# KorAP/Datok

Measured on AMD Instinct MI355X. Metric: input MB/s tokenized, tokenizer_de.matok, higher is better.
Workload: dtype u32 table cells, u8 symbol codes; 1 GPU; tokenizer_de.matok, 4096 equal-length 4096 B synthetic German docs per batch (BASELINE.json configs[1]); table_layout=matrix: state-major fused u32 cells, docs_per_gpu=4096, doc_bytes=4096, parallelism=documents sharded over 1 GPU(s), no data-path collective, batches_in_flight=3, inputs=one per batch in flight (generator seeds 2, 3, 4 on rank 0)

## Files before the change

### datok_amd/_lib.py

```python
import ctypes as C
import os
import subprocess

_HERE = os.path.dirname(os.path.abspath(__file__))
LIB_PATH = os.environ.get("DATOK_GPU_LIB") or os.path.join(_HERE, "libdatok_gpu.so")

OK, E_IO, E_FORMAT, E_NO_DEVICE, E_HIP, E_ARG, E_MODEL, E_CAPACITY, E_STATE, E_NOMEM = 0, -1, -2, -3, -4, -5, -6, -7, -8, -9
ST_WINDOW_OVERFLOW, ST_EMPTY_TEXT, ST_BAD_MODEL, ST_IRREGULAR, ST_STEP_LIMIT, ST_INTERNAL = 1, 2, 4, 8, 16, 32
ST_BAD_OFFSET = 64

EXPORTS = [
    "dtk_device_count", "dtk_set_device", "dtk_strerror", "dtk_last_hip_error",
    "dtk_model_load", "dtk_model_load_mem", "dtk_model_free", "dtk_model_type", "dtk_model_get_info",
    "dtk_model_info_mem",
    "dtk_batch_create", "dtk_batch_free", "dtk_batch_set_input", "dtk_batch_set_input_device",
    "dtk_batch_run", "dtk_batch_sync", "dtk_batch_stream", "dtk_batch_totals",
    "dtk_batch_set_profiling", "dtk_batch_stage_ms", "dtk_batch_set_chunking", "dtk_batch_set_warm_extend",
    "dtk_batch_result_device", "dtk_batch_result_host", "dtk_transduce", "dtk_free",
    "dtk_foma_to_matok", "dtk_foma_to_datok", "dtk_transduce_replay", "dtk_batch_render_device", "dtk_batch_render_host",
    "dtk_batch_status_host", "dtk_transduce_release", "dtk_transduce_result",
    "dtk_pipeline_create", "dtk_pipeline_free", "dtk_pipeline_set_chunking", "dtk_pipeline_run",
    "dtk_pinned_alloc", "dtk_pinned_free",
    "dtk_batch_set_result_fields", "dtk_batch_download_begin", "dtk_pipeline_set_result_fields",
    "dtk_batch_set_download_stream", "dtk_batch_download_stream", "dtk_batch_done", "dtk_batch_set_streams",
    "dtk_debug_configure", "dtk_batch_debug_stream", "dtk_blk_start", "dtk_blk_end",
    "dtk_multi_create", "dtk_multi_free", "dtk_multi_type", "dtk_multi_set_result_fields", "dtk_multi_set_chunking", "dtk_multi_run",
]


class ModelInfo(C.Structure):
    _fields_ = [("kind", C.c_int32), ("epsilon", C.c_int32), ("unknown", C.c_int32),
                ("identity", C.c_int32), ("final_state", C.c_int32), ("sigma_count", C.c_int32),
                ("state_count", C.c_uint32), ("array_len", C.c_uint64),
                ("n_eps_states", C.c_uint32), ("max_eps_chain", C.c_uint32),
                ("entry_bytes", C.c_uint32), ("device_bytes", C.c_uint64),
                ("unknown_used", C.c_uint32), ("dense_states", C.c_uint32),
                ("stream_codes", C.c_uint32)]


class Totals(C.Structure):
# ... 117 lines not shown
    L.dtk_multi_free.argtypes = [vp]
    L.dtk_multi_free.restype = None
    L.dtk_multi_type.argtypes = [vp]
    L.dtk_multi_type.restype = C.c_char_p
    L.dtk_multi_set_result_fields.argtypes = [vp, u32]
    L.dtk_multi_set_chunking.argtypes = [vp, u32, u32]
    L.dtk_multi_run.argtypes = [vp, vp, vp, u32, u32, SLICE_FN, vp]
    for f in (L.dtk_blk_start, L.dtk_blk_end):
        f.argtypes, f.restype = [vp, vp, u64], C.c_int32
    L.dtk_pinned_alloc.restype = vp
    L.dtk_pinned_alloc.argtypes = [sz]
    L.dtk_pinned_free.argtypes = [vp]
    L.dtk_pinned_free.restype = None
    L.dtk_debug_configure.argtypes = [C.c_char_p, C.c_char_p]
    L.dtk_batch_debug_stream.argtypes = [vp, vp, vp, C.POINTER(u32)]
    for k, v in os.environ.items():
        if k.startswith("DATOK_") and k not in ("DATOK_GPU_LIB", "DATOK_GATHER_TIMEOUT"):
            L.dtk_debug_configure(k.encode(), v.encode())
    _lib = L
    return L


def check(code, what=""):
    if code != OK:
        raise DatokGpuError(code, what)
```

### datok_amd/csrc/dtk_batch.cpp

```cpp
#include <algorithm>
#include <cstdio>
#include <cstring>
#include <memory>

#include "dtk_host.h"

static int alloc_outputs(dtk_batch *b, uint64_t tok, uint64_t sent, uint64_t text) {
  auto grow = [](auto &a, uint64_t n) { return a.fit(n, std::max<uint64_t>(n, 4)); };
  int rc;
  if (tok > b->tok_cap) {
    b->tok_cap = 0;
    if ((rc = grow(b->d_rstart, tok)) || (rc = grow(b->d_rend, tok)) || (rc = grow(b->d_bstart, tok)) ||
        (rc = grow(b->d_bend, tok)) || (rc = grow(b->d_sbefore, tok)))
      return rc;
    b->tok_cap = tok;
  }
  if (sent > b->sent_cap) {
    b->sent_cap = 0;
    if ((rc = grow(b->d_sent, sent))) return rc;
    b->sent_cap = sent;
  }
  if (text > b->text_cap) {
    b->text_cap = 0;
    if ((rc = grow(b->d_ttok, text)) || (rc = grow(b->d_tsent, text)) || (rc = grow(b->d_ts_end, text))) return rc;
// ... 6 lines not shown
  if (!out || max_docs == 0) return DTK_E_ARG;
  *out = nullptr;
  if (dtk_device_count() <= 0) return DTK_E_NO_DEVICE;
  std::unique_ptr<dtk_batch> b(new dtk_batch());
  b->max_bytes = max_bytes;
  b->max_docs = max_docs;
  HIP_TRY(hipGetDevice(&b->device));
  int rc = b->stream.create();
  if (rc != DTK_OK) return rc;
  if (g_dbg.round_limit >= 0) b->round_limit = (uint32_t)g_dbg.round_limit;
  const uint64_t pad = 256, nd1 = (uint64_t)max_docs + 1;
  auto make = [](auto &a, uint64_t n) { return a.fit(n, n); };
  if ((rc = make(b->d_text_own, max_bytes + pad)) || (rc = make(b->d_off_own, nd1)) ||
      (rc = make(b->d_sym, max_bytes + pad)) || (rc = make(b->d_rsbits, (max_bytes + pad) / 8 + 64)) ||
      (rc = make(b->d_bits, EVB_KINDS * ((max_bytes + max_docs) / 32 + 8) + 8)) ||
      (rc = make(b->d_acc, DTK_TOTALS_BYTES + 3 * nd1 * 8 + 4 * (uint64_t)max_docs * 4 + 64)) ||
      (rc = make(b->d_redo, max_docs)) || (rc = make(b->d_blk_doc, max_bytes / DTK_SYM_BLOCK_BYTES + 3)) ||
      (rc = make(b->d_chunk_off, nd1)) || (rc = make(b->d_big_docs, nd1)) ||
      (rc = make(b->d_csr, 3 * nd1)) || (rc = make(b->d_doc_ns, nd1)) ||
      (rc = make(b->d_scan_ws, ((uint64_t)max_docs / 2048 + 2) * 4)) || (rc = make(b->d_out_off, nd1)) ||
      (rc = b->h_totals_pin.fit(DTK_TOTALS_BYTES, DTK_TOTALS_BYTES)) || (rc = b->h_off_pin.fit(nd1 * 8, nd1 * 8)))
    return rc;
  b->d_tok_off = b->d_csr; b->d_sent_off = b->d_csr + nd1; b->d_text_off = b->d_csr + 2 * nd1;
  b->h_totals = b->h_totals_pin.as<DtkTotalsDev>();
  rc = alloc_outputs(b.get(), max_bytes / 3 + max_docs + 16, max_bytes / 8 + 2ull * max_docs + 16,
                     max_bytes / 64 + 2ull * max_docs + 16);
  if (rc != DTK_OK) return rc;
  *out = b.release();
  return DTK_OK;
}

// ... 307 lines not shown
  }
  b->last_model = m;
  b->last_flags = flags;
  b->repair_rounds = 0;
  hipStream_t s = b->stream;
  const bool prof = b->profiling;
#define STAGE(i) do { if (prof) HIP_TRY(hipEventRecord(b->ev[i], s)); } while (0)
  STAGE(0);
  bool fold_acc = false;
  size_t acc_bytes = 0;
  {
    const size_t nd = b->n_docs;
    uint8_t *q = b->d_acc;
    b->d_tok_off = b->d_csr; b->d_sent_off = b->d_csr + (nd + 1); b->d_text_off = b->d_csr + 2 * (nd + 1);
    b->d_totals = (DtkTotalsDev *)q; q += DTK_TOTALS_BYTES;
    b->d_tok_cnt = (uint64_t *)q; q += (nd + 1) * 8;
    b->d_sent_cnt = (uint64_t *)q; q += (nd + 1) * 8;
    b->d_text_cnt = (uint64_t *)q; q += (nd + 1) * 8;
    b->d_status = (uint32_t *)q; q += nd * 4;
    b->d_first_bad = (uint32_t *)q; q += nd * 4;
    b->d_fail_lane = (uint32_t *)q; q += nd * 4;
    b->d_doc_tail = (uint32_t *)q; q += nd * 4;
    const size_t acc_used = ((size_t)(q - b->d_acc) + 15) & ~(size_t)15;
    b->bit_words = (uint32_t)(((b->total + nd) / 32 + 8) & ~(uint64_t)3);
    const bool fold = b->total > 0;
    fold_acc = fold && b->acc_primed && acc_used / 16 < 0xFFFFFFFFull && !g_dbg.clear_kernel;
    if (!fold_acc) {
      if (dtk_launch_clear2(b->d_acc, acc_used, b->d_bits, fold ? 0 : (size_t)EVB_KINDS * b->bit_words * 4, s))
        return hip_fail(hipGetLastError(), "clear");
      b->acc_primed = true;
    }
    acc_bytes = acc_used;
  }
  STAGE(1);
  if (dtk_launch_symbolize(b->d_text, b->d_off, b->n_docs, b->total, &m->sig, b->d_sym,
                           b->d_text == b->d_text_own, b->d_blk_doc, (unsigned long long *)&b->d_totals->invalid_epoch,
                           (uint32_t *)b->d_rsbits.p, b->d_bits, b->bit_words, fold_acc ? b->d_acc.p : nullptr, acc_bytes,
                           ++b->epoch, s))
    return hip_fail(hipGetLastError(), "symbolize");
  STAGE(2);
  DtkWalkArgs w = walk_args(b);
  bool fix_in_scan = false;
  DtkSpecArgs sp_first{};
  if (b->chunk == 0) {
    STAGE(3); STAGE(4);
    if (dtk_launch_walk(&m->tab, &w, s)) return hip_fail(hipGetLastError(), "walk");
    STAGE(5); STAGE(6); STAGE(7);
  } else {
    DtkSpecArgs sp = spec_args(b, false);
    sp_first = sp;
    uint32_t *nb = b->d_totals->n_bad;
    const bool split = g_dbg.split_start != 0 || sp.lds_words == 0;
    b->dev_rounds = g_dbg.dev_rounds >= 0 ? (uint32_t)g_dbg.dev_rounds : (b->expect_repairs ? 2u : 0u);
    if (b->dev_rounds > 3u) b->dev_rounds = 3u;
    fix_in_scan = b->n_docs <= 8192u && b->dev_rounds == 0;
#define SPEC(stage)                                                                               \
  do {                                                                                            \
    if (dtk_launch_spec(&m->tab, &w, &sp, stage, cmp_mask_of(m), b->d_redo, nb, s))               \
      return hip_fail(hipGetLastError(), "speculative walk");                                     \
  } while (0)
    if (split) {
      SPEC(0); STAGE(3); SPEC(1); STAGE(4); SPEC(2); STAGE(5); SPEC(3); STAGE(6);
    } else {
      STAGE(3); STAGE(4); SPEC(6); STAGE(5); SPEC(7); STAGE(6);
    }
    if (!fix_in_scan) SPEC(4);
    STAGE(7);
#undef SPEC
    for (uint32_t r = 0; r < b->dev_rounds; r++) {
      DtkSpecArgs rp = spec_args(b, true);
      rp.go = nb + r;
      int rc = repair_round(b, m, &w, &rp, nb + r + 1);
      if (rc != DTK_OK) return rc;
    }
  }
  DtkCompactArgs c{};
  c.text = b->d_text; c.rs_bits = (const uint32_t *)b->d_rsbits.p; c.doc_off = b->d_off; c.n_docs = b->n_docs;
  c.bits = b->d_bits; c.bit_words = b->bit_words; c.doc_tail = b->d_doc_tail; c.status = b->d_status;
  c.flags = flags & DTK_NEWLINE_AFTER_EOT; c.kind = m->kind;
  c.totals = &b->d_totals->n_tok;
  if (dtk_launch_scan3(b->d_tok_cnt, b->d_sent_cnt, b->d_text_cnt, b->d_tok_off, b->d_sent_off, b->d_text_off,
                       b->n_docs, &b->d_totals->n_tok, b->d_status, b->d_scan_ws, fix_in_scan ? &sp_first : nullptr, b->d_redo,
                       b->d_totals->n_bad, b->chunk ? n_bad_now(b) : nullptr, s))
    return hip_fail(hipGetLastError(), "scan");
  STAGE(8);
  c.skip_if = b->chunk ? n_bad_now(b) : nullptr;
  b->last_args = c;
  b->ran_full = false;
  const bool eager_full = g_dbg.compact_full != 0;
  int rc = launch_compact2(b, (b->expect_eot || eager_full) ? 3 : 1);
  if (rc != DTK_OK) return rc;
  STAGE(9);
#undef STAGE
  b->eager_fields = 0;
  b->results_changed = false;
  if (b->fields & DTK_R_EAGER) {
    rc = launch_to_host(b);
    if (rc != DTK_OK) return rc;
  }
// ... 87 lines not shown
  if (!b->ran) return DTK_E_STATE;
  if (b->totals_valid) return DTK_OK;
  { const int rc_ = wait_own(b); if (rc_ != DTK_OK) return rc_; }
  if (b->chunk != 0) {
    const uint32_t *hnb = b->h_totals->n_bad;
    for (uint32_t r = 0; r < b->dev_rounds; r++)
      if (hnb[r] != 0) b->repair_rounds++;
    uint32_t left = hnb[b->dev_rounds];
    if (left != 0) {
      b->results_changed = true;
      const dtk_model *m = b->last_model;
      hipStream_t s = b->stream;
      DtkWalkArgs w = walk_args(b);
      uint32_t *n_bad = n_bad_now(b);
      const uint32_t max_rounds = b->max_doc_lanes + 16u;
      while (left != 0) {
        b->repair_rounds++;
        DtkSpecArgs sp = spec_args(b, true);
        HIP_TRY(hipMemsetAsync(n_bad, 0, 4, s));
        int rc = repair_round(b, m, &w, &sp, n_bad);
        if (rc != DTK_OK) return rc;
        HIP_TRY(hipMemcpyAsync(&left, n_bad, 4, hipMemcpyDeviceToHost, s));
        HIP_TRY(hipStreamSynchronize(s));
        if (left != 0 && g_dbg.debug_repair && b->repair_rounds < 12) {
          std::vector<uint32_t> redo(b->n_docs), chunk_off(b->n_docs + 1);
          HIP_TRY(hipMemcpy(redo.data(), b->d_redo, (size_t)b->n_docs * 4, hipMemcpyDeviceToHost));
          HIP_TRY(hipMemcpy(chunk_off.data(), b->d_chunk_off, ((size_t)b->n_docs + 1) * 4, hipMemcpyDeviceToHost));
          for (uint32_t d = 0, shown = 0; d < b->n_docs && shown < 3; d++)
            if (redo[d] != 0xFFFFFFFFu) {
              const uint32_t L0 = chunk_off[d], L1 = chunk_off[d + 1], n = std::min<uint32_t>(L1 - L0, 24u);
// ... 10 lines not shown
        if (left != 0 && (b->repair_rounds > max_rounds || b->repair_rounds >= b->round_limit)) {
          const uint32_t rounds = b->repair_rounds, keep = b->cfg_chunk;
          b->cfg_chunk = 0; b->plan_valid = false;
          rc = dtk_batch_run(m, b, b->last_flags);
          if (rc == DTK_OK) rc = finish(b);
          b->cfg_chunk = keep; b->plan_valid = false;
          b->repair_rounds = rounds; b->totals.repair_rounds = rounds;
          b->expect_repairs = true;
          return rc;
        }
      }
      if (dtk_launch_scan3(b->d_tok_cnt, b->d_sent_cnt, b->d_text_cnt, b->d_tok_off, b->d_sent_off, b->d_text_off,
                         b->n_docs, &b->d_totals->n_tok, b->d_status, b->d_scan_ws, nullptr, nullptr, nullptr, nullptr, s))
        return hip_fail(hipGetLastError(), "scan");
      b->last_args.skip_if = nullptr;
      int rc = launch_compact2(b, 3);
      if (rc != DTK_OK) return rc;
      HIP_TRY(hipMemcpyAsync(b->h_totals, b->d_totals, DTK_TOTALS_BYTES, hipMemcpyDeviceToHost, s));
      HIP_TRY(hipStreamSynchronize(s));
    }
    b->expect_repairs = b->repair_rounds != 0;
  }
  const uint64_t nt = b->h_totals->n_tok, ns = b->h_totals->n_sent, nx = b->h_totals->n_text;
  b->n_invalid = b->h_totals->invalid_epoch == b->epoch ? 1u : 0u;
  if (nt > b->tok_cap || ns > b->sent_cap || nx > b->text_cap) {
    b->results_changed = true;
    int rc = alloc_outputs(b, nt + nt / 8 + 16, ns + ns / 8 + 16, nx + nx / 8 + 16);
    if (rc != DTK_OK) return rc;
    if ((rc = launch_compact2(b, 3)) != DTK_OK || (rc = reread_flags(b)) != DTK_OK) return rc;
  }
// ... 67 lines not shown
    for (uint32_t c = 0; c <= DTK_SYM_MASK; c++) sym_of_col[c] = (uint16_t)c;
    for (size_t a = 0; a < m->col.size(); a++)
      if (m->col[a] <= DTK_SYM_MASK) sym_of_col[m->col[a]] = (uint16_t)a;
    for (size_t i = 0; i < n; i++)
      entries[i] = (uint16_t)((entries[i] & ~DTK_SYM_MASK) | sym_of_col[entries[i] & DTK_SYM_MASK]);
  }
  if (rune_start_words && n)
    HIP_TRY(hipMemcpy(rune_start_words, b->d_rsbits.p, (n + 31) / 32 * sizeof(uint32_t), hipMemcpyDeviceToHost));
  if (saw_invalid) {
    uint64_t seen = 0;
    HIP_TRY(hipMemcpy(&seen, &b->d_totals->invalid_epoch, sizeof seen, hipMemcpyDeviceToHost));
    *saw_invalid = (n && seen == b->epoch) ? 1u : 0u;
  }
  return DTK_OK;
}
```

### datok_amd/csrc/dtk_compact.hip

```cpp
#include "dtk_device.h"


#define CQ_CAP 512u
#define CT_CAP 512u

struct SegRange { uint32_t d, p0, p1; bool first, last; };
__device__ __forceinline__ bool seg_range(const DtkCompactArgs &A, uint32_t s, uint32_t len_of_d, SegRange &r) {
  const uint32_t La = A.seg_lane0[s], Lb = La + A.seg_nl[s];
  const uint32_t L0 = A.chunk_off[r.d], L1 = A.chunk_off[r.d + 1];
  r.first = La == L0;
  r.last = Lb >= L1;
  r.p0 = r.first ? 0u : A.lane_start[La].p;
  if (r.p0 == 0xFFFFFFFFu) return false;
  r.p1 = r.last ? len_of_d : A.lane_start[Lb].p;
  if (r.p1 == 0xFFFFFFFFu) { r.p1 = len_of_d; r.last = true; }
  return true;
}

__device__ __forceinline__ uint32_t bits32(const uint32_t *__restrict__ b, uint32_t bit) {
  const uint32_t w = bit >> 5, sh = bit & 31u;
  const uint32_t lo = b[w], hi = b[w + 1];
  return (uint32_t)((((uint64_t)hi << 32) | lo) >> sh);
}
__device__ __forceinline__ uint32_t lowmask(uint32_t n) { return n >= 32u ? 0xFFFFFFFFu : (1u << n) - 1u; }

#ifdef DTK_PROBE
__device__ unsigned long long g_cphase[8];
extern "C" int dtk_cphase_read(unsigned long long *out, int reset) {
  hipDeviceSynchronize();
  hipMemcpyFromSymbol(out, HIP_SYMBOL(g_cphase), sizeof(g_cphase));
  if (reset) { unsigned long long z[8] = {0}; hipMemcpyToSymbol(HIP_SYMBOL(g_cphase), z, sizeof(z)); }
  return 0;
}
#define CPROBE(i) do { if (!FULL) { const unsigned long long n_ = clock64(); pr_c[i] += n_ - pr_last; pr_last = n_; } } while (0)
#else
#define CPROBE(i) do { } while (0)
#endif

template <bool FULL>
__device__ __forceinline__ void compact_unit(const DtkCompactArgs &A, uint32_t small_max, const uint32_t *big_docs) {
  __shared__ uint32_t qpos[FULL ? CQ_CAP : 1u], qrn[FULL ? CQ_CAP : 1u], qst[FULL ? CQ_CAP : 1u], qsr[FULL ? CQ_CAP : 1u];
  __shared__ uint8_t qfl[FULL ? CQ_CAP : 1u];
  __shared__ uint2 s_tok[CT_CAP];
  __shared__ uint16_t s_sb[CT_CAP];
#ifdef DTK_PROBE
  unsigned long long pr_c[8] = {0, 0, 0, 0, 0, 0, 0, 0}, pr_last = clock64();
#endif
  const bool seg_mode = A.seg_doc != nullptr;
  const uint32_t d = (uint32_t)__builtin_amdgcn_readfirstlane(
      (int)(seg_mode ? A.seg_doc[blockIdx.x] : (big_docs ? big_docs[blockIdx.x] : blockIdx.x)));
  const uint32_t skip_now = A.skip_if ? *A.skip_if : 0u;
  const uint64_t off = A.doc_off[d], off_end = A.doc_off[d + 1];
  const uint32_t st_d = A.status[d], tail_d = A.doc_tail[d];
  const uint64_t tot0 = A.totals[0], tot1 = A.totals[1], tot2 = A.totals[2];
  const uint64_t tok_base = A.tok_off[d], sent_base = A.sent_off[d], text_base = A.text_off[d];
  const uint64_t tok_lim = A.tok_off[d + 1], sent_lim = A.sent_off[d + 1], text_lim = A.text_off[d + 1];
  if (skip_now != 0u) return;
  const uint32_t len = (uint32_t)(off_end - off);
  if (len <= small_max && small_max != 0u) return;
  const uint32_t gb = (uint32_t)DTK_EV_BIT(off, d);
  const uint32_t *__restrict__ bE = A.bits + (size_t)EVB_END * A.bit_words;
  const uint32_t *__restrict__ bS = A.bits + (size_t)EVB_START * A.bit_words;
  const uint32_t *__restrict__ bP = A.bits + (size_t)EVB_SEPS * A.bit_words;
  const uint32_t *__restrict__ bT = A.bits + (size_t)EVB_TEOT * A.bit_words;
  const uint32_t *__restrict__ bU = A.bits + (size_t)EVB_SEOT * A.bit_words;
  const uint8_t *__restrict__ txt = A.text + off;
  const bool nl_rule = (A.flags & 16u) != 0;
  const bool is_matrix = A.kind == DTK_KIND_MATRIX;
  const uint32_t lane = lane_id();
  const unsigned long long lt = lanemask_lt();
  if (st_d & ST_IRREGULAR) {
    if (lane == 0) atomicOr(A.any_irregular, 1u);
// ... 969 lines not shown
```

### datok_amd/csrc/dtk_device.h

```cpp
#pragma once
#include <hip/hip_runtime.h>
#include <stdint.h>

#include <type_traits>

#include "dtk_internal.h"

#define WAVE 64
#ifndef DTK_WARM_TAG
#define DTK_WARM_TAG 64u
#endif


__device__ __forceinline__ uint32_t lane_id() { return threadIdx.x & (WAVE - 1); }
__device__ __forceinline__ unsigned long long lanemask_lt() { return (1ull << lane_id()) - 1ull; }
__device__ __forceinline__ int highest(unsigned long long m) { return 63 - __clzll((long long)m); }
__device__ __forceinline__ uint32_t popc(unsigned long long m) { return (uint32_t)__popcll(m); }

__device__ __forceinline__ uint32_t wave_excl_scan(uint32_t v, uint32_t &total) {
  uint32_t x = v;
  x += (uint32_t)__builtin_amdgcn_update_dpp(0, (int)x, 0x111, 0xF, 0xF, true);
  x += (uint32_t)__builtin_amdgcn_update_dpp(0, (int)x, 0x112, 0xF, 0xF, true);
  x += (uint32_t)__builtin_amdgcn_update_dpp(0, (int)x, 0x114, 0xF, 0xF, true);
  x += (uint32_t)__builtin_amdgcn_update_dpp(0, (int)x, 0x118, 0xF, 0xF, true);
  x += (uint32_t)__builtin_amdgcn_update_dpp(0, (int)x, 0x142, 0xA, 0xF, false);
  x += (uint32_t)__builtin_amdgcn_update_dpp(0, (int)x, 0x143, 0xC, 0xF, false);
  total = (uint32_t)__builtin_amdgcn_readlane((int)x, WAVE - 1);
  return x - v;
}

#define DTK_WAVE_FOLD(x, op)                                                                   \
  do {                                                                                         \
    x = op(x, __builtin_amdgcn_update_dpp(x, x, 0x111, 0xF, 0xF, false));       \
    x = op(x, __builtin_amdgcn_update_dpp(x, x, 0x112, 0xF, 0xF, false));       \
    x = op(x, __builtin_amdgcn_update_dpp(x, x, 0x114, 0xF, 0xF, false));       \
    x = op(x, __builtin_amdgcn_update_dpp(x, x, 0x118, 0xF, 0xF, false));       \
    x = op(x, __builtin_amdgcn_update_dpp(x, x, 0x142, 0xA, 0xF, false));    \
    x = op(x, __builtin_amdgcn_update_dpp(x, x, 0x143, 0xC, 0xF, false));    \
  } while (0)
__device__ __forceinline__ int32_t wave_min(int32_t v) {
  int x = v;
  DTK_WAVE_FOLD(x, min);
  return __builtin_amdgcn_readlane(x, WAVE - 1);
// ... 13 lines not shown
  return lo;
}

__device__ __forceinline__ void mark_redo(const DtkSpecArgs &S, uint32_t d, uint32_t bad, uint32_t *redo_out,
                                          uint32_t *n_bad) {
  const uint32_t L0 = S.chunk_off[d], L1 = S.chunk_off[d + 1];
  DtkLaneState en = S.lane_end[bad];
  en.flags &= (LANE_F_SENT | LANE_F_TEXT | LANE_F_OK);
  if (en.p != 0xFFFFFFFFu && bad + 1 < L1) S.lane_start[bad + 1] = en;
  uint32_t r0 = bad;
  if (bad > L0) {
    r0 = bad - 1u;
    while (r0 > L0 && S.lane_end[r0].p == S.lane_start[r0].p) r0--;
  }
  redo_out[d] = r0;
  atomicAdd(n_bad, 1u);
}
```

### datok_amd/csrc/dtk_host.h

```cpp
#pragma once
#include <hip/hip_runtime.h>

#include <string>
#include <type_traits>
#include <vector>

#include "../../include/datok_gpu.h"
#include "dtk_internal.h"
#include "dtk_own.h"

#pragma GCC visibility push(hidden)

struct DtkDebug {
  int sym16 = 0;
  int force_wide = 0;
  int file_columns = 0;
  int no_fused = 0;
  int wide_fused = 0;
  int no_dense = 0;
  int small_max = -1;
  int lds_bits = 1;
  int split_start = 0;
  int dev_rounds = -1;
  int compact_full = 0;
// ... 70 lines not shown
  bool long_docs = false;
  uint32_t max_doc_lanes = 0;
  DevArray<uint32_t> d_blk_doc;
  uint32_t small_max = 0, n_big = 0;
  DevArray<uint32_t> d_big_docs;
  uint32_t *d_first_bad = nullptr, *d_fail_lane = nullptr;
  DevArray<DtkLaneCount> d_lane_cnt;
  DevArray<DtkLaneState> d_lane_start, d_lane_end;
  DevArray<DtkLanePlan> d_lane_plan;
  uint32_t repair_rounds = 0;
  const dtk_model *last_model = nullptr;
  uint32_t last_flags = 0;
  DevArray<uint64_t> d_csr;
  uint64_t *d_tok_off = nullptr, *d_sent_off = nullptr, *d_text_off = nullptr;
  uint64_t *d_tok_cnt = nullptr, *d_sent_cnt = nullptr, *d_text_cnt = nullptr;
  DevArray<uint64_t> d_scan_ws;
  DtkTotalsDev *d_totals = nullptr;
  uint32_t dev_rounds = 0;
  bool expect_repairs = false;
  uint32_t round_limit = 0xFFFFFFFFu;
  bool acc_primed = false;
  uint64_t epoch = 0;
  bool expect_eot = false;
  bool ran_full = false;
  PinBuf h_totals_pin;
  DtkTotalsDev *h_totals = nullptr;
  PinBuf h_off_pin;
  uint64_t tok_cap = 0, sent_cap = 0, text_cap = 0;
  DevArray<int32_t> d_rstart, d_rend, d_sent;
  DevArray<uint32_t> d_bstart, d_bend, d_ttok, d_tsent;
// ... 83 lines not shown
```

### datok_amd/csrc/dtk_internal.h

```cpp
#pragma once
#include <stddef.h>
#include <stdint.h>

#define DTK_FIRSTBIT 0x80000000u
#define DTK_SECONDBIT 0x40000000u
#define DTK_RESTBIT 0x3fffffffu
#define DTK_EOT 4u
#define DTK_WINDOW 1024u
#define DTK_WINDOW_BYTES 4104u

#define DTK_SYM_MASK 0x7FFu
#define DTK_SYM_MAX 2047u
#define DTK_SYM_W_SHIFT 11
#define DTK_SYM_CLS_SHIFT 14
#define DTK_SYM_WIDTH(e) (((uint32_t)(e) >> DTK_SYM_W_SHIFT) & 7u)
#define DTK_SYM_IS_START(e) (DTK_SYM_WIDTH(e) != 0u)
#define DTK_WIN 32u
#define DTK_WIN_ROW 36u
#define DTK_SYM_CONT 0xFFu
#ifndef DTK_WIN8
#define DTK_WIN8 32u
#endif
struct DtkSym {
  const void *base;
// ... 56 lines not shown
  uint64_t invalid_epoch;
  uint32_t any_irregular, any_eot;
  uint32_t n_bad[4];
  uint64_t render_total;
  uint64_t to_host_epoch;
  uint64_t unused_12[4];
};
static_assert(sizeof(struct DtkTotalsDev) == DTK_TOTALS_BYTES - DTK_STEP_STRIPES * 128u, "the block is 128 bytes");
static_assert(offsetof(struct DtkTotalsDev, n_tok) == 0 && offsetof(struct DtkTotalsDev, n_sent) == 8 &&
              offsetof(struct DtkTotalsDev, n_text) == 16 && offsetof(struct DtkTotalsDev, n_flagged) == 24,
              "the scan's four totals are the first four words");
static_assert(offsetof(struct DtkTotalsDev, invalid_epoch) % 16 == 0 &&
              offsetof(struct DtkTotalsDev, any_irregular) == offsetof(struct DtkTotalsDev, invalid_epoch) + 8,
              "invalid_epoch and the two flags share a 16-byte unit");
static inline uint64_t *dtk_step_stripe(struct DtkTotalsDev *t, uint32_t i) { return (uint64_t *)(t + 1) + 16u * i; }

struct DtkTableDev {
  int kind;
  const void *tab;
  uint32_t entry_bytes;
  uint32_t stride;
  uint32_t n_states;
  uint32_t n_eps;
  uint32_t start;
  uint32_t fused;
  uint32_t ident_guard;
  uint32_t da_dense;
  uint32_t da_len;
  uint32_t da_size;
  uint32_t da_base1;
// ... 43 lines not shown
  uint32_t lds_words;
  const uint32_t *go;
};

struct DtkWalkArgs {
  struct DtkSym sym;
  const uint64_t *doc_off;
  uint32_t n_docs;
  uint32_t *bits;
  uint32_t bit_words;
  uint32_t *doc_tail;
  uint32_t *status;
  uint64_t *tok_cnt, *sent_cnt, *text_cnt;
  unsigned long long *steps;
  uint32_t step_factor;
};

struct DtkCompactArgs {
  const uint8_t *text;
  const uint32_t *rs_bits;
  const uint64_t *doc_off;
  uint32_t n_docs;
  const uint32_t *bits;
  uint32_t bit_words;
  const uint32_t *doc_tail;
  uint32_t *status;
  uint32_t flags;
  int kind;
  uint64_t *tok_off, *sent_off, *text_off;
  int32_t *tok_rstart, *tok_rend;
  uint32_t *tok_bstart, *tok_bend;
  int32_t *sent;
  uint32_t *text_tok_end, *text_sent_end;
  uint32_t *tok_sbefore, *text_s_end, *doc_ns;
  const uint64_t *totals;
  uint64_t tok_cap, sent_cap, text_cap;
  const uint32_t *seg_doc, *seg_lane0, *seg_nl;
  uint32_t n_segs;
  const uint32_t *chunk_off;
  const struct DtkLaneState *lane_start;
  const struct DtkLaneCount *lane_cnt;
  struct DtkSegSum *seg_sum;
  struct DtkSegIn *seg_in;
  uint32_t *doc_seq;
  uint32_t *any_irregular;
  uint32_t *any_eot;
  const uint32_t *skip_if;
};

#define DTK_SEG_LANES 64u
// ... 137 lines not shown
```

### datok_amd/csrc/dtk_repair.hip

```cpp
#include "dtk_device.h"

__global__ __launch_bounds__(256) void k_spec_link(DtkSpecArgs S) {
  if (S.go && *S.go == 0u) return;
  const uint32_t L = blockIdx.x * blockDim.x + threadIdx.x;
  if (L >= S.n_lanes) return;
  const uint32_t d = S.lane_doc[L];
  const uint32_t L0 = S.chunk_off[d], L1 = S.chunk_off[d + 1];
  bool linked = false;
  if (L + 1 < L1) {
    const uint32_t np = S.lane_start[L + 1].p, mp = S.lane_start[L].p;
    linked = np != 0xFFFFFFFFu && mp != 0xFFFFFFFFu && np >= mp;
  }
  if (!linked) atomicMax(&S.first_bad[d], ~(L - L0));
}

#define VERIFY_TB 256u
__global__ __launch_bounds__(VERIFY_TB) void k_spec_verify(DtkWalkArgs A, DtkSpecArgs S, uint32_t cmp_mask, uint32_t local_link) {
  if (S.go && *S.go == 0u) return;
  const uint32_t L = blockIdx.x * blockDim.x + threadIdx.x;
  bool live = L < S.n_lanes;
  uint32_t d = 0xFFFFFFFFu;
  DtkLaneCount c{0u, 0u, 0u, 0u, 0u, 0xFFFFFFFFu, 0u, 0u};
  if (live) {
    d = S.lane_doc[L];
    if (S.redo_from && S.redo_from[d] == 0xFFFFFFFFu) { live = false; d = 0xFFFFFFFFu; }
  }
  if (live && local_link) {
    const uint32_t L0 = S.chunk_off[d], L1 = S.chunk_off[d + 1];
    const bool has_next = L + 1u < L1;
    const DtkLaneState own = S.lane_start[L], en = S.lane_end[L];
    DtkLaneState nx{0xFFFFFFFFu, 0u, 0u, 0u};
    if (has_next) nx = S.lane_start[L + 1];
    uint32_t link_ok = 1u;
    if (own.p == 0xFFFFFFFFu) {
      if (nx.p != 0xFFFFFFFFu) {
        uint32_t x = L - 1u;
        while (x > L0 && S.lane_start[x].p == 0xFFFFFFFFu) x--;
        atomicMax(&S.fail_lane[d], ~x);
      }
    } else {
      bool good;
      if (nx.p != 0xFFFFFFFFu && nx.p >= own.p) {
        good = en.p == nx.p && en.t == nx.t && ((en.flags ^ nx.flags) & cmp_mask) == 0 && !(en.flags & LANE_F_DROPPED);
      } else {
        good = nx.p == 0xFFFFFFFFu && en.p == 0xFFFFFFFFu && !(en.flags & LANE_F_IDLE);
      }
      if (good) c = S.lane_cnt[L]; else atomicMax(&S.fail_lane[d], ~L);
      link_ok = good ? 1u : 0u;
    }
    S.lane_plan[L].pad = link_ok;
  } else if (live) {
    const uint32_t L0 = S.chunk_off[d];
    const uint32_t k = L - L0, fb = ~S.first_bad[d];
    uint32_t link_ok = 1u;
    if (k > fb) {
      if (S.lane_start[L].p != 0xFFFFFFFFu) atomicMax(&S.fail_lane[d], ~(L0 + fb));
    } else {
      const DtkLaneState en = S.lane_end[L];
      bool good;
      if (k < fb) {
        const DtkLaneState nx = S.lane_start[L + 1];
        good = en.p == nx.p && en.t == nx.t && ((en.flags ^ nx.flags) & cmp_mask) == 0 &&
               !(en.flags & LANE_F_DROPPED);
      } else {
        good = en.p == 0xFFFFFFFFu && !(en.flags & LANE_F_IDLE);
      }
      if (good) c = S.lane_cnt[L]; else atomicMax(&S.fail_lane[d], ~L);
      link_ok = good ? 1u : 0u;
    }
    S.lane_plan[L].pad = link_ok;
  }
  uint32_t tok = c.tok, sent = c.sent, text = c.text, st = c.status;
#pragma unroll
  for (int o = 1; o < WAVE; o <<= 1) {
    const uint32_t dn = __shfl_down(d, o);
    const uint32_t t2 = __shfl_down(tok, o), s2 = __shfl_down(sent, o), x2 = __shfl_down(text, o),
                   st2 = __shfl_down(st, o);
    const bool same = (lane_id() + o < WAVE) && dn == d;
    tok += same ? t2 : 0u; sent += same ? s2 : 0u; text += same ? x2 : 0u; st |= same ? st2 : 0u;
  }
  const uint32_t dprev = __shfl_up(d, 1);
  const bool head = live && (lane_id() == 0 || dprev != d);
  __shared__ uint32_t s_d[VERIFY_TB / WAVE], s_v[VERIFY_TB / WAVE][4];
  const uint32_t wid = threadIdx.x >> 6;
  const bool whole = __ballot(head) == 1ull;
  if (lane_id() == 0) {
    s_d[wid] = whole ? d : 0xFFFFFFFFu;
    s_v[wid][0] = tok; s_v[wid][1] = sent; s_v[wid][2] = text; s_v[wid][3] = st;
  }
  __syncthreads();
  bool merged = s_d[0] != 0xFFFFFFFFu;
#pragma unroll
  for (uint32_t w = 1; w < VERIFY_TB / WAVE; w++) merged = merged && s_d[w] == s_d[0];
  if (merged) {
    if (threadIdx.x == 0) {
      uint32_t a0 = 0, a1 = 0, a2 = 0, a3 = 0;
      for (uint32_t w = 0; w < VERIFY_TB / WAVE; w++) { a0 += s_v[w][0]; a1 += s_v[w][1]; a2 += s_v[w][2]; a3 |= s_v[w][3]; }
      if (a0) atomicAdd((unsigned long long *)&A.tok_cnt[d], (unsigned long long)a0);
      if (a1) atomicAdd((unsigned long long *)&A.sent_cnt[d], (unsigned long long)a1);
      if (a2) atomicAdd((unsigned long long *)&A.text_cnt[d], (unsigned long long)a2);
      if (a3) atomicOr(&A.status[d], a3);
    }
  } else if (head) {
    if (tok) atomicAdd((unsigned long long *)&A.tok_cnt[d], (unsigned long long)tok);
    if (sent) atomicAdd((unsigned long long *)&A.sent_cnt[d], (unsigned long long)sent);
    if (text) atomicAdd((unsigned long long *)&A.text_cnt[d], (unsigned long long)text);
    if (st) atomicOr(&A.status[d], st);
  }
}

__global__ __launch_bounds__(256) void k_spec_fix(DtkWalkArgs A, DtkSpecArgs S, uint32_t *redo_out,
                                                  uint32_t *n_bad) {
  if (S.go && *S.go == 0u) return;
  const uint32_t d = blockIdx.x * blockDim.x + threadIdx.x;
  if (d >= A.n_docs) return;
  const uint32_t bad = ~S.fail_lane[d];
  if (bad == 0xFFFFFFFFu) { redo_out[d] = 0xFFFFFFFFu; return; }
  mark_redo(S, d, bad, redo_out, n_bad);
}

__global__ __launch_bounds__(256) void k_redo_spread(DtkSpecArgs S) {
  if (S.go && *S.go == 0u) return;
// ... 101 lines not shown
```

### datok_amd/host.py

```python
import ctypes as C
import io
import sys

import numpy as np

from . import _lib
from ._lib import ModelInfo, RenderView, ResultView, Totals, check, lib

TOKENS, SENTENCES, TOKEN_POS, SENTENCE_POS, NEWLINE_AFTER_EOT = 1, 2, 4, 8, 16
SIMPLE = TOKENS | SENTENCES
OFFSETS_ONLY, NO_BYTE_OFFSETS, NO_RUNE_OFFSETS = 256, 512, 1024

EV_S_EOT, EV_E_EOT, EV_TOK_END, EV_S_EPS, EV_S_EOF, EV_E_EOF = 1, 2, 4, 8, 32, 64
EVB_END, EVB_START, EVB_SEPS, EVB_TEOT, EVB_SEOT = 0, 1, 2, 3, 4
EVL_SEOT, EVL_TEOT, EVL_SEPS = 1, 2, 4


def _decode_runes(b: bytes):
    out, i, n = [], 0, len(b)
    while i < n:
        b0 = b[i]
        r, w = 0xFFFD, 1
        if b0 < 0x80:
            r = b0
# ... 378 lines not shown
        return dict(zip(self.STAGES, [float(x) for x in ms]))

    def totals(self):
        t = Totals()
        check(lib().dtk_batch_totals(self._h, C.byref(t)), "dtk_batch_totals")
        return {k: getattr(t, k) for k, _ in Totals._fields_}

    def debug_stream(self):
        entries = np.zeros(self.total, dtype=np.uint16)
        words = np.zeros((self.total + 31) // 32, dtype=np.uint32)
        saw = C.c_uint32(0)
        check(lib().dtk_batch_debug_stream(self._h, entries.ctypes.data, words.ctypes.data, C.byref(saw)),
              "dtk_batch_debug_stream")
        return entries, words, bool(saw.value)

    def result_device(self) -> ResultView:
        v = ResultView()
        check(lib().dtk_batch_result_device(self._h, C.byref(v)), "dtk_batch_result_device")
        return v

    def render_device(self, flags=SIMPLE) -> RenderView:
        v = RenderView()
        check(lib().dtk_batch_render_device(self._h, flags, C.byref(v)), "dtk_batch_render_device")
        return v

    def render(self, flags=SIMPLE):
        v = RenderView()
        check(lib().dtk_batch_render_host(self._h, flags, C.byref(v)), "dtk_batch_render_host")
        off = np.frombuffer((C.c_char * ((self.n_docs + 1) * 8)).from_address(v.doc_off), dtype=np.uint64).copy()
        data = C.string_at(v.bytes, v.total) if v.total else b""
# ... 196 lines not shown
```

### include/datok_gpu.h

```cpp
#ifndef DATOK_GPU_H
#define DATOK_GPU_H

#include <stddef.h>
#include <stdint.h>

#ifdef __cplusplus
extern "C" {
#endif

enum {
  DTK_OK = 0,
  DTK_E_IO = -1,
  DTK_E_FORMAT = -2,
  DTK_E_NO_DEVICE = -3,
  DTK_E_HIP = -4,
  DTK_E_ARG = -5,
  DTK_E_MODEL = -6,
  DTK_E_CAPACITY = -7,
  DTK_E_STATE = -8,
  DTK_E_NOMEM = -9
};

enum {
  DTK_TOKENS = 1,
// ... 29 lines not shown
  return ((uint32_t)(i & 63u) < h->brk ? h->base0 : h->base1) + (int32_t)(words[i] & 0xFFFFu);
}
DTK_BLK_DECODER int32_t dtk_blk_end(const uint32_t *words, const dtk_off_block *heads, uint64_t i) {
  const dtk_off_block *h = heads + (i >> 6);
  return ((uint32_t)(i & 63u) < h->brk ? h->base0 : h->base1) + (int32_t)(words[i] >> 16);
}

int dtk_device_count(void);
int dtk_set_device(int device);
const char *dtk_strerror(int code);
const char *dtk_last_hip_error(void);

int dtk_debug_configure(const char *key, const char *value);

int dtk_batch_debug_stream(dtk_batch *b, uint16_t *entries, uint32_t *rune_start_words, uint32_t *saw_invalid);

int dtk_model_load(const char *path, dtk_model **out);
int dtk_model_load_mem(const void *gz_bytes, size_t n, dtk_model **out);
void dtk_model_free(dtk_model *m);
int dtk_foma_to_matok(const void *gz_bytes, size_t n, void **out, size_t *out_n);
int dtk_foma_to_datok(const void *gz_bytes, size_t n, void **out, size_t *out_n);
const char *dtk_model_type(const dtk_model *m);

typedef struct {
  int32_t kind;
  int32_t epsilon, unknown, identity, final_state, sigma_count;
  uint32_t state_count;
  uint64_t array_len;
  uint32_t n_eps_states;
  uint32_t max_eps_chain;
// ... 146 lines not shown
```

Before: 170,600 MB/s.

## Fold per-document row offset scan into compaction via per-group count totals

For batches of up to 8192 docs without repair rounds, the verify kernel now also accumulates per-64-doc group totals of token/sentence/text counts, and the compaction kernel derives each document's base offsets with wave-level 64-bit sums instead of relying on a separate scan3 launch and spec stage 4. Compaction writes the CSR offsets and totals itself, and the repair path re-launches stage 4 only when needed. This removes one or two kernel launches and a global scan pass from the common path. The cost is extra atomics on group counters and redundant per-wave reductions in every compaction unit.

```diff
diff --git a/datok_amd/_lib.py b/datok_amd/_lib.py
--- a/datok_amd/_lib.py
+++ b/datok_amd/_lib.py
@@ -23,7 +23,7 @@
     "dtk_pinned_alloc", "dtk_pinned_free",
     "dtk_batch_set_result_fields", "dtk_batch_download_begin", "dtk_pipeline_set_result_fields",
     "dtk_batch_set_download_stream", "dtk_batch_download_stream", "dtk_batch_done", "dtk_batch_set_streams",
-    "dtk_debug_configure", "dtk_batch_debug_stream", "dtk_blk_start", "dtk_blk_end",
+    "dtk_debug_configure", "dtk_batch_debug_stream", "dtk_batch_debug_rows_in_compaction", "dtk_blk_start", "dtk_blk_end",
     "dtk_multi_create", "dtk_multi_free", "dtk_multi_type", "dtk_multi_set_result_fields", "dtk_multi_set_chunking", "dtk_multi_run",
 ]
 
@@ -171,6 +171,7 @@
     L.dtk_pinned_free.restype = None
     L.dtk_debug_configure.argtypes = [C.c_char_p, C.c_char_p]
     L.dtk_batch_debug_stream.argtypes = [vp, vp, vp, C.POINTER(u32)]
+    L.dtk_batch_debug_rows_in_compaction.argtypes = [vp]
     for k, v in os.environ.items():
         if k.startswith("DATOK_") and k not in ("DATOK_GPU_LIB", "DATOK_GATHER_TIMEOUT"):
             L.dtk_debug_configure(k.encode(), v.encode())
diff --git a/datok_amd/csrc/dtk_batch.cpp b/datok_amd/csrc/dtk_batch.cpp
--- a/datok_amd/csrc/dtk_batch.cpp
+++ b/datok_amd/csrc/dtk_batch.cpp
@@ -44,7 +44,7 @@
   if ((rc = make(b->d_text_own, max_bytes + pad)) || (rc = make(b->d_off_own, nd1)) ||
       (rc = make(b->d_sym, max_bytes + pad)) || (rc = make(b->d_rsbits, (max_bytes + pad) / 8 + 64)) ||
       (rc = make(b->d_bits, EVB_KINDS * ((max_bytes + max_docs) / 32 + 8) + 8)) ||
-      (rc = make(b->d_acc, DTK_TOTALS_BYTES + 3 * nd1 * 8 + 4 * (uint64_t)max_docs * 4 + 64)) ||
+      (rc = make(b->d_acc, DTK_TOTALS_BYTES + 3 * DTK_ROW_GROUPS * 8 + 3 * nd1 * 8 + 4 * (uint64_t)max_docs * 4 + 64)) ||
       (rc = make(b->d_redo, max_docs)) || (rc = make(b->d_blk_doc, max_bytes / DTK_SYM_BLOCK_BYTES + 3)) ||
       (rc = make(b->d_chunk_off, nd1)) || (rc = make(b->d_big_docs, nd1)) ||
       (rc = make(b->d_csr, 3 * nd1)) || (rc = make(b->d_doc_ns, nd1)) ||
@@ -382,6 +382,7 @@
     uint8_t *q = b->d_acc;
     b->d_tok_off = b->d_csr; b->d_sent_off = b->d_csr + (nd + 1); b->d_text_off = b->d_csr + 2 * (nd + 1);
     b->d_totals = (DtkTotalsDev *)q; q += DTK_TOTALS_BYTES;
+    b->d_grp_cnt = (uint64_t *)q; q += 3 * DTK_ROW_GROUPS * 8;
     b->d_tok_cnt = (uint64_t *)q; q += (nd + 1) * 8;
     b->d_sent_cnt = (uint64_t *)q; q += (nd + 1) * 8;
     b->d_text_cnt = (uint64_t *)q; q += (nd + 1) * 8;
@@ -408,7 +409,7 @@
     return hip_fail(hipGetLastError(), "symbolize");
   STAGE(2);
   DtkWalkArgs w = walk_args(b);
-  bool fix_in_scan = false;
+  bool fix_in_scan = false, rows_here = false;
   DtkSpecArgs sp_first{};
   if (b->chunk == 0) {
     STAGE(3); STAGE(4);
@@ -421,7 +422,9 @@
     const bool split = g_dbg.split_start != 0 || sp.lds_words == 0;
     b->dev_rounds = g_dbg.dev_rounds >= 0 ? (uint32_t)g_dbg.dev_rounds : (b->expect_repairs ? 2u : 0u);
     if (b->dev_rounds > 3u) b->dev_rounds = 3u;
-    fix_in_scan = b->n_docs <= 8192u && b->dev_rounds == 0;
+    rows_here = b->n_docs <= 64u * DTK_ROW_GROUPS && b->dev_rounds == 0 && b->small_max == 0 && !b->long_docs;
+    if (rows_here) { w.grp_cnt = b->d_grp_cnt; w.n_flagged = &b->d_totals->n_flagged; w.n_broken = nb; }
+    fix_in_scan = !rows_here && b->n_docs <= 8192u && b->dev_rounds == 0;
 #define SPEC(stage)                                                                               \
   do {                                                                                            \
     if (dtk_launch_spec(&m->tab, &w, &sp, stage, cmp_mask_of(m), b->d_redo, nb, s))               \
@@ -432,7 +435,7 @@
     } else {
       STAGE(3); STAGE(4); SPEC(6); STAGE(5); SPEC(7); STAGE(6);
     }
-    if (!fix_in_scan) SPEC(4);
+    if (!fix_in_scan && !rows_here) SPEC(4);
     STAGE(7);
 #undef SPEC
     for (uint32_t r = 0; r < b->dev_rounds; r++) {
@@ -447,10 +450,14 @@
   c.bits = b->d_bits; c.bit_words = b->bit_words; c.doc_tail = b->d_doc_tail; c.status = b->d_status;
   c.flags = flags & DTK_NEWLINE_AFTER_EOT; c.kind = m->kind;
   c.totals = &b->d_totals->n_tok;
-  if (dtk_launch_scan3(b->d_tok_cnt, b->d_sent_cnt, b->d_text_cnt, b->d_tok_off, b->d_sent_off, b->d_text_off,
-                       b->n_docs, &b->d_totals->n_tok, b->d_status, b->d_scan_ws, fix_in_scan ? &sp_first : nullptr, b->d_redo,
-                       b->d_totals->n_bad, b->chunk ? n_bad_now(b) : nullptr, s))
+  b->rows_in_compaction = rows_here;
+  if (rows_here) {
+    c.grp_cnt = b->d_grp_cnt; c.tok_cnt = b->d_tok_cnt; c.sent_cnt = b->d_sent_cnt; c.text_cnt = b->d_text_cnt;
+  } else if (dtk_launch_scan3(b->d_tok_cnt, b->d_sent_cnt, b->d_text_cnt, b->d_tok_off, b->d_sent_off, b->d_text_off,
+                              b->n_docs, &b->d_totals->n_tok, b->d_status, b->d_scan_ws, fix_in_scan ? &sp_first : nullptr,
+                              b->d_redo, b->d_totals->n_bad, b->chunk ? n_bad_now(b) : nullptr, s)) {
     return hip_fail(hipGetLastError(), "scan");
+  }
   STAGE(8);
   c.skip_if = b->chunk ? n_bad_now(b) : nullptr;
   b->last_args = c;
@@ -568,6 +575,11 @@
       DtkWalkArgs w = walk_args(b);
       uint32_t *n_bad = n_bad_now(b);
       const uint32_t max_rounds = b->max_doc_lanes + 16u;
+      if (b->rows_in_compaction) {
+        DtkSpecArgs sp = spec_args(b, false);
+        if (dtk_launch_spec(&m->tab, &w, &sp, 4, cmp_mask_of(m), b->d_redo, nullptr, s))
+          return hip_fail(hipGetLastError(), "speculative repair");
+      }
       while (left != 0) {
         b->repair_rounds++;
         DtkSpecArgs sp = spec_args(b, true);
@@ -608,6 +620,7 @@
                          b->n_docs, &b->d_totals->n_tok, b->d_status, b->d_scan_ws, nullptr, nullptr, nullptr, nullptr, s))
         return hip_fail(hipGetLastError(), "scan");
       b->last_args.skip_if = nullptr;
+      b->last_args.grp_cnt = nullptr;
       int rc = launch_compact2(b, 3);
       if (rc != DTK_OK) return rc;
       HIP_TRY(hipMemcpyAsync(b->h_totals, b->d_totals, DTK_TOTALS_BYTES, hipMemcpyDeviceToHost, s));
@@ -705,3 +718,8 @@
   }
   return DTK_OK;
 }
+
+extern "C" int dtk_batch_debug_rows_in_compaction(dtk_batch *b) {
+  if (!b || !b->ran) return DTK_E_ARG;
+  return b->rows_in_compaction ? 1 : 0;
+}
diff --git a/datok_amd/csrc/dtk_compact.hip b/datok_amd/csrc/dtk_compact.hip
--- a/datok_amd/csrc/dtk_compact.hip
+++ b/datok_amd/csrc/dtk_compact.hip
@@ -36,6 +36,28 @@
 #else
 #define CPROBE(i) do { } while (0)
 #endif
+
+struct DocRows { uint64_t base[3], lim[3], tot[3]; };
+__device__ __forceinline__ void rows_from_counts(const DtkCompactArgs &A, uint32_t d, DocRows &R) {
+  const uint32_t lane = lane_id(), g = d >> 6, di = (g << 6) + lane;
+  const uint32_t dc = di < A.n_docs ? di : d;
+  const uint64_t *cnt[3] = {A.tok_cnt, A.sent_cnt, A.text_cnt};
+  uint64_t g0[3], g1[3], c[3], own[3];
+#pragma unroll
+  for (int j = 0; j < 3; j++) {
+    g0[j] = A.grp_cnt[(uint32_t)j * DTK_ROW_GROUPS + lane];
+    g1[j] = A.grp_cnt[(uint32_t)j * DTK_ROW_GROUPS + 64u + lane];
+    c[j] = cnt[j][dc];
+    own[j] = cnt[j][d];
+  }
+#pragma unroll
+  for (int j = 0; j < 3; j++) {
+    const uint64_t below = (lane < g ? g0[j] : 0ull) + (lane + 64u < g ? g1[j] : 0ull) + (di < d ? c[j] : 0ull);
+    R.base[j] = wave_sum64(below);
+    R.lim[j] = R.base[j] + own[j];
+    R.tot[j] = wave_sum64(g0[j] + g1[j]);
+  }
+}
 
 template <bool FULL>
 __device__ __forceinline__ void compact_unit(const DtkCompactArgs &A, uint32_t small_max, const uint32_t *big_docs) {
@@ -52,10 +74,25 @@
   const uint32_t skip_now = A.skip_if ? *A.skip_if : 0u;
   const uint64_t off = A.doc_off[d], off_end = A.doc_off[d + 1];
   const uint32_t st_d = A.status[d], tail_d = A.doc_tail[d];
-  const uint64_t tot0 = A.totals[0], tot1 = A.totals[1], tot2 = A.totals[2];
-  const uint64_t tok_base = A.tok_off[d], sent_base = A.sent_off[d], text_base = A.text_off[d];
-  const uint64_t tok_lim = A.tok_off[d + 1], sent_lim = A.sent_off[d + 1], text_lim = A.text_off[d + 1];
+  DocRows R;
+  if (A.grp_cnt) {
+    rows_from_counts(A, d, R);
+  } else {
+    R.tot[0] = A.totals[0]; R.tot[1] = A.totals[1]; R.tot[2] = A.totals[2];
+    R.base[0] = A.tok_off[d]; R.base[1] = A.sent_off[d]; R.base[2] = A.text_off[d];
+    R.lim[0] = A.tok_off[d + 1]; R.lim[1] = A.sent_off[d + 1]; R.lim[2] = A.text_off[d + 1];
+  }
+  const uint64_t tot0 = R.tot[0], tot1 = R.tot[1], tot2 = R.tot[2];
+  const uint64_t tok_base = R.base[0], sent_base = R.base[1], text_base = R.base[2];
+  const uint64_t tok_lim = R.lim[0], sent_lim = R.lim[1], text_lim = R.lim[2];
   if (skip_now != 0u) return;
+  if (A.grp_cnt && lane_id() == 0u) {
+    A.tok_off[d] = tok_base; A.sent_off[d] = sent_base; A.text_off[d] = text_base;
+    if (d + 1u == A.n_docs) {
+      A.tok_off[d + 1] = tot0; A.sent_off[d + 1] = tot1; A.text_off[d + 1] = tot2;
+      A.totals[0] = tot0; A.totals[1] = tot1; A.totals[2] = tot2;
+    }
+  }
   const uint32_t len = (uint32_t)(off_end - off);
   if (len <= small_max && small_max != 0u) return;
   const uint32_t gb = (uint32_t)DTK_EV_BIT(off, d);
diff --git a/datok_amd/csrc/dtk_device.h b/datok_amd/csrc/dtk_device.h
--- a/datok_amd/csrc/dtk_device.h
+++ b/datok_amd/csrc/dtk_device.h
@@ -27,6 +27,25 @@
   x += (uint32_t)__builtin_amdgcn_update_dpp(0, (int)x, 0x143, 0xC, 0xF, false);
   total = (uint32_t)__builtin_amdgcn_readlane((int)x, WAVE - 1);
   return x - v;
+}
+
+__device__ __forceinline__ uint64_t wave_sum64(uint64_t v) {
+#define DTK_SUM64_STEP(ctrl, rows, bound)                                                                    \
+  do {                                                                                                       \
+    const uint32_t lo_ = (uint32_t)__builtin_amdgcn_update_dpp(0, (int)(uint32_t)v, ctrl, rows, 0xF, bound); \
+    const uint32_t hi_ = (uint32_t)__builtin_amdgcn_update_dpp(0, (int)(v >> 32), ctrl, rows, 0xF, bound);   \
+    v += ((uint64_t)hi_ << 32) | lo_;                                                                        \
+  } while (0)
+  DTK_SUM64_STEP(0x111, 0xF, true);
+  DTK_SUM64_STEP(0x112, 0xF, true);
+  DTK_SUM64_STEP(0x114, 0xF, true);
+  DTK_SUM64_STEP(0x118, 0xF, true);
+  DTK_SUM64_STEP(0x142, 0xA, false);
+  DTK_SUM64_STEP(0x143, 0xC, false);
+#undef DTK_SUM64_STEP
+  const uint32_t lo = (uint32_t)__builtin_amdgcn_readlane((int)(uint32_t)v, WAVE - 1);
+  const uint32_t hi = (uint32_t)__builtin_amdgcn_readlane((int)(v >> 32), WAVE - 1);
+  return ((uint64_t)hi << 32) | lo;
 }
 
 #define DTK_WAVE_FOLD(x, op)                                                                   \
@@ -70,5 +89,5 @@
     while (r0 > L0 && S.lane_end[r0].p == S.lane_start[r0].p) r0--;
   }
   redo_out[d] = r0;
-  atomicAdd(n_bad, 1u);
+  if (n_bad) atomicAdd(n_bad, 1u);
 }
diff --git a/datok_amd/csrc/dtk_host.h b/datok_amd/csrc/dtk_host.h
--- a/datok_amd/csrc/dtk_host.h
+++ b/datok_amd/csrc/dtk_host.h
@@ -108,6 +108,8 @@
   DevArray<uint64_t> d_csr;
   uint64_t *d_tok_off = nullptr, *d_sent_off = nullptr, *d_text_off = nullptr;
   uint64_t *d_tok_cnt = nullptr, *d_sent_cnt = nullptr, *d_text_cnt = nullptr;
+  uint64_t *d_grp_cnt = nullptr;
+  bool rows_in_compaction = false;
   DevArray<uint64_t> d_scan_ws;
   DtkTotalsDev *d_totals = nullptr;
   uint32_t dev_rounds = 0;
diff --git a/datok_amd/csrc/dtk_internal.h b/datok_amd/csrc/dtk_internal.h
--- a/datok_amd/csrc/dtk_internal.h
+++ b/datok_amd/csrc/dtk_internal.h
@@ -94,6 +94,8 @@
               offsetof(struct DtkTotalsDev, any_irregular) == offsetof(struct DtkTotalsDev, invalid_epoch) + 8,
               "invalid_epoch and the two flags share a 16-byte unit");
 static inline uint64_t *dtk_step_stripe(struct DtkTotalsDev *t, uint32_t i) { return (uint64_t *)(t + 1) + 16u * i; }
+
+#define DTK_ROW_GROUPS 128u
 
 struct DtkTableDev {
   int kind;
@@ -167,6 +169,9 @@
   uint64_t *tok_cnt, *sent_cnt, *text_cnt;
   unsigned long long *steps;
   uint32_t step_factor;
+  uint64_t *grp_cnt;
+  uint64_t *n_flagged;
+  uint32_t *n_broken;
 };
 
 struct DtkCompactArgs {
@@ -186,7 +191,9 @@
   int32_t *sent;
   uint32_t *text_tok_end, *text_sent_end;
   uint32_t *tok_sbefore, *text_s_end, *doc_ns;
-  const uint64_t *totals;
+  uint64_t *totals;
+  const uint64_t *grp_cnt;
+  const uint64_t *tok_cnt, *sent_cnt, *text_cnt;
   uint64_t tok_cap, sent_cap, text_cap;
   const uint32_t *seg_doc, *seg_lane0, *seg_nl;
   uint32_t n_segs;
diff --git a/datok_amd/csrc/dtk_repair.hip b/datok_amd/csrc/dtk_repair.hip
--- a/datok_amd/csrc/dtk_repair.hip
+++ b/datok_amd/csrc/dtk_repair.hip
@@ -21,6 +21,9 @@
   bool live = L < S.n_lanes;
   uint32_t d = 0xFFFFFFFFu;
   DtkLaneCount c{0u, 0u, 0u, 0u, 0u, 0xFFFFFFFFu, 0u, 0u};
+  auto fail = [&](uint32_t lane_inv) {
+    if (atomicMax(&S.fail_lane[d], lane_inv) == 0u && A.n_broken) atomicAdd(A.n_broken, 1u);
+  };
   if (live) {
     d = S.lane_doc[L];
     if (S.redo_from && S.redo_from[d] == 0xFFFFFFFFu) { live = false; d = 0xFFFFFFFFu; }
@@ -36,7 +39,7 @@
       if (nx.p != 0xFFFFFFFFu) {
         uint32_t x = L - 1u;
         while (x > L0 && S.lane_start[x].p == 0xFFFFFFFFu) x--;
-        atomicMax(&S.fail_lane[d], ~x);
+        fail(~x);
       }
     } else {
       bool good;
@@ -45,7 +48,7 @@
       } else {
         good = nx.p == 0xFFFFFFFFu && en.p == 0xFFFFFFFFu && !(en.flags & LANE_F_IDLE);
       }
-      if (good) c = S.lane_cnt[L]; else atomicMax(&S.fail_lane[d], ~L);
+      if (good) c = S.lane_cnt[L]; else fail(~L);
       link_ok = good ? 1u : 0u;
     }
     S.lane_plan[L].pad = link_ok;
@@ -54,7 +57,7 @@
     const uint32_t k = L - L0, fb = ~S.first_bad[d];
     uint32_t link_ok = 1u;
     if (k > fb) {
-      if (S.lane_start[L].p != 0xFFFFFFFFu) atomicMax(&S.fail_lane[d], ~(L0 + fb));
+      if (S.lane_start[L].p != 0xFFFFFFFFu) fail(~(L0 + fb));
     } else {
       const DtkLaneState en = S.lane_end[L];
       bool good;
@@ -65,7 +68,7 @@
       } else {
         good = en.p == 0xFFFFFFFFu && !(en.flags & LANE_F_IDLE);
       }
-      if (good) c = S.lane_cnt[L]; else atomicMax(&S.fail_lane[d], ~L);
+      if (good) c = S.lane_cnt[L]; else fail(~L);
       link_ok = good ? 1u : 0u;
     }
     S.lane_plan[L].pad = link_ok;
@@ -81,31 +84,58 @@
   }
   const uint32_t dprev = __shfl_up(d, 1);
   const bool head = live && (lane_id() == 0 || dprev != d);
-  __shared__ uint32_t s_d[VERIFY_TB / WAVE], s_v[VERIFY_TB / WAVE][4];
+  __shared__ uint32_t s_d[VERIFY_TB / WAVE], s_v[VERIFY_TB / WAVE][4], s_g[VERIFY_TB / WAVE][3];
   const uint32_t wid = threadIdx.x >> 6;
   const bool whole = __ballot(head) == 1ull;
+  bool one_group = false;
+  uint32_t grp = 0;
+  if (A.grp_cnt) {
+    const uint32_t Lb = blockIdx.x * blockDim.x, Le = min(Lb + blockDim.x, S.n_lanes) - 1u;
+    grp = S.lane_doc[Lb] >> 6;
+    one_group = grp == (S.lane_doc[Le] >> 6);
+  }
+  if (one_group) {
+    uint32_t wt, ws, wx;
+    (void)wave_excl_scan(c.tok, wt); (void)wave_excl_scan(c.sent, ws); (void)wave_excl_scan(c.text, wx);
+    if (lane_id() == 0) { s_g[wid][0] = wt; s_g[wid][1] = ws; s_g[wid][2] = wx; }
+  }
   if (lane_id() == 0) {
     s_d[wid] = whole ? d : 0xFFFFFFFFu;
     s_v[wid][0] = tok; s_v[wid][1] = sent; s_v[wid][2] = text; s_v[wid][3] = st;
   }
   __syncthreads();
+  if (one_group && threadIdx.x == 0) {
+    unsigned long long *g = (unsigned long long *)A.grp_cnt + grp;
+#pragma unroll
+    for (uint32_t j = 0; j < 3u; j++) {
+      uint32_t a = 0;
+      for (uint32_t w = 0; w < VERIFY_TB / WAVE; w++) a += s_g[w][j];
+      if (a) atomicAdd(g + j * DTK_ROW_GROUPS, (unsigned long long)a);
+    }
+  }
   bool merged = s_d[0] != 0xFFFFFFFFu;
 #pragma unroll
   for (uint32_t w = 1; w < VERIFY_TB / WAVE; w++) merged = merged && s_d[w] == s_d[0];
+  auto add = [&](uint32_t t, uint32_t s, uint32_t x, uint32_t stat) {
+    if (t) atomicAdd((unsigned long long *)&A.tok_cnt[d], (unsigned long long)t);
+    if (s) atomicAdd((unsigned long long *)&A.sent_cnt[d], (unsigned long long)s);
+    if (x) atomicAdd((unsigned long long *)&A.text_cnt[d], (unsigned long long)x);
+    if (A.grp_cnt && !one_group) {
+      unsigned long long *g = (unsigned long long *)A.grp_cnt + (d >> 6);
+      if (t) atomicAdd(g, (unsigned long long)t);
+      if (s) atomicAdd(g + DTK_ROW_GROUPS, (unsigned long long)s);
+      if (x) atomicAdd(g + 2u * DTK_ROW_GROUPS, (unsigned long long)x);
+    }
+    if (stat && atomicOr(&A.status[d], stat) == 0u && A.n_flagged) atomicAdd((unsigned long long *)A.n_flagged, 1ull);
+  };
   if (merged) {
     if (threadIdx.x == 0) {
       uint32_t a0 = 0, a1 = 0, a2 = 0, a3 = 0;
       for (uint32_t w = 0; w < VERIFY_TB / WAVE; w++) { a0 += s_v[w][0]; a1 += s_v[w][1]; a2 += s_v[w][2]; a3 |= s_v[w][3]; }
-      if (a0) atomicAdd((unsigned long long *)&A.tok_cnt[d], (unsigned long long)a0);
-      if (a1) atomicAdd((unsigned long long *)&A.sent_cnt[d], (unsigned long long)a1);
-      if (a2) atomicAdd((unsigned long long *)&A.text_cnt[d], (unsigned long long)a2);
-      if (a3) atomicOr(&A.status[d], a3);
+      add(a0, a1, a2, a3);
     }
   } else if (head) {
-    if (tok) atomicAdd((unsigned long long *)&A.tok_cnt[d], (unsigned long long)tok);
-    if (sent) atomicAdd((unsigned long long *)&A.sent_cnt[d], (unsigned long long)sent);
-    if (text) atomicAdd((unsigned long long *)&A.text_cnt[d], (unsigned long long)text);
-    if (st) atomicOr(&A.status[d], st);
+    add(tok, sent, text, st);
   }
 }
 
diff --git a/datok_amd/host.py b/datok_amd/host.py
--- a/datok_amd/host.py
+++ b/datok_amd/host.py
@@ -416,6 +416,12 @@
               "dtk_batch_debug_stream")
         return entries, words, bool(saw.value)
 
+    def debug_rows_in_compaction(self):
+        r = lib().dtk_batch_debug_rows_in_compaction(self._h)
+        if r < 0:
+            raise _lib.DatokGpuError(r, "dtk_batch_debug_rows_in_compaction")
+        return bool(r)
+
     def result_device(self) -> ResultView:
         v = ResultView()
         check(lib().dtk_batch_result_device(self._h, C.byref(v)), "dtk_batch_result_device")
diff --git a/include/datok_gpu.h b/include/datok_gpu.h
--- a/include/datok_gpu.h
+++ b/include/datok_gpu.h
@@ -67,6 +67,8 @@
 int dtk_debug_configure(const char *key, const char *value);
 
 int dtk_batch_debug_stream(dtk_batch *b, uint16_t *entries, uint32_t *rune_start_words, uint32_t *saw_invalid);
+
+int dtk_batch_debug_rows_in_compaction(dtk_batch *b);
 
 int dtk_model_load(const char *path, dtk_model **out);
 int dtk_model_load_mem(const void *gz_bytes, size_t n, dtk_model **out);
```

Result: faster. 173,600 MB/s (median of 6 runs) (+1.8%).
